# mukteshkrmishra/namazu

Measured on AMD Instinct MI355X. Metric: schedule decisions/sec + trace-pair edit distances/sec at 1/2/4/8 MI355X, higher is better.
Workload: dtype u64; 1 GPU; configs[1] replayable seed sweep; seeds_per_gpu=1048576, events=4096, max_interval_ns=100000000, topk=64, pipeline_streams=3, parallelism=seed-range x1

## Files before the change

### namazu_amd/csrc/replayable.hip

```cpp
#include <algorithm>
#include <cstring>
#include <cstdlib>
#include <numeric>
#include <string>
#include <vector>

#include "nmz_common.h"
#include "nmz_internal.h"
#include "replayable_plan.h"

namespace nmz {

__global__ __launch_bounds__(256) void k_replayable_table(const uint32_t *__restrict__ hoff,
                                                          const uint8_t *__restrict__ hbytes,
                                                          const uint32_t *__restrict__ perm, uint32_t E,
                                                          uint64_t m, int fast, uint4 *__restrict__ table) {
    const uint32_t pos = blockIdx.x;
    const uint32_t L = threadIdx.x;
    const uint32_t e = perm[pos];
    const uint32_t b0 = hoff[e], b1 = hoff[e + 1];
    uint64_t h = L;
    for (uint32_t i = b0; i < b1; ++i) h = fnv_step(h, hbytes[i]);
    const uint64_t C = h - (uint64_t)L * fnv_pow(b1 - b0);
    const uint32_t cm = fast ? (uint32_t)(C % m) : 0u;
// ... 172 lines not shown
    uint64_t h = FNV_OFFSET;
    for (uint32_t i = soff[s], end = soff[s + 1]; i < end; ++i) h = fnv_step(h, sbytes[i]);
    for (uint32_t i = hoff[e], end = hoff[e + 1]; i < end; ++i) h = fnv_step(h, hbytes[i]);
    out[idx] = m ? (int64_t)(h % m) : 0;
}

static bool use_wt(const nmz_replayable_plan *p) {
    return p->wt.on && (replay_oq_enabled() || p->mod.kind != MOD_FAST);
}
static bool use_oq(const nmz_replayable_plan *p) {
    return p->oq.on && (replay_oq_enabled() || p->mod.kind != MOD_FAST);
}

static bool wt_topk_enabled() {
    static const bool on = [] {
        const char *e = ab_env("NMZ_WT_TOPK");
        return !(e && std::string(e) == "0");
    }();
    return on;
}

static int replayable_stats(nmz_replayable_plan *p, hipStream_t st, const uint32_t *d_soff,
                            const uint8_t *d_sbytes, uint64_t S, nmz_sched_stats *d_stats, uint64_t dec_lo = 0,
                            void *wt_topk_scratch = nullptr, uint32_t k = 0,
                            const nmz_replayable_seeds *pre = nullptr) {
    if (S == 0) return NMZ_OK;
    const uint32_t E = p->n_events;
    if (E == 0 || p->mod.kind == MOD_ZERO) {
        hipLaunchKernelGGL(k_stats_constant, dim3(ceil_div(S, 256)), dim3(256), 0, st, S, E, d_stats);
        NMZ_HIP(hipGetLastError());
        return NMZ_OK;
    }
    const bool wt = use_wt(p), stats_kernel = wt || use_oq(p);
    SeedScratch sc;
    if (pre && stats_kernel) {
        sc = pre->sc;
    } else {
        NMZ_CHECK(S <= p->max_seeds, "more seeds than the plan was created for");
        sc = carve_seed_scratch(p->seed_scratch.ptr, p->max_seeds);
        if (pre) {
            NMZ_HIP(hipMemcpyAsync(sc.b.hist, pre->hist, bucket_hist_u32(S) * sizeof(uint32_t),
                                   hipMemcpyDeviceToDevice, st));
            sc.h0 = pre->sc.h0;
        } else {
            NMZ_TRY(seed_prefix_launch(st, d_soff, d_sbytes, dec_lo, S, sc.h0, sc.b.hist));
        }
        if (stats_kernel) NMZ_TRY(bucket_seeds_counted(st, sc.h0, S, OQ_WG, sc.b, sc.counter));
    }
    if (wt) return wt_sweep(p->wt, p->ctx, st, sc.b, p->d_table, E, p->mod, d_stats, S, wt_topk_scratch, k);
    if (stats_kernel) return oq_sweep(p->oq, p->ctx, st, sc.b, p->d_table, E, p->mod, d_stats);
    return pd_sweep(p, st, sc, S, d_stats);
}

static int replayable_run_on(nmz_replayable_plan *p, hipStream_t st, const uint32_t *d_soff, const uint8_t *d_sbytes,
                             uint64_t S, nmz_sched_stats *d_stats, uint64_t seed0, uint32_t k, nmz_topk_entry *d_topk,
                             uint64_t dec_lo, const nmz_replayable_seeds *pre);

static int replayable_run(nmz_replayable_plan *p, hipStream_t st, const uint32_t *d_soff, const uint8_t *d_sbytes,
                          uint64_t S, nmz_sched_stats *d_stats, uint64_t seed0 = 0, uint32_t k = 0,
                          nmz_topk_entry *d_topk = nullptr, uint64_t dec_lo = 0,
                          const nmz_replayable_seeds *pre = nullptr) {
    nmz_replayable_plan::Use *u = nullptr;
    for (auto &x : p->uses)
        if (x.st == st) u = &x;
    if (!u) {
        hipEvent_t ev;
        NMZ_HIP(hipEventCreateWithFlags(&ev, hipEventDisableTiming));
        p->uses.push_back({st, ev});
        u = &p->uses.back();
        if (p->built && st != p->ctx->stream) NMZ_HIP(hipStreamWaitEvent(st, p->built, 0));
    }
    const int rc = replayable_run_on(p, st, d_soff, d_sbytes, S, d_stats, seed0, k, d_topk, dec_lo, pre);
// ... 2 lines not shown
}

static void plan_wait_uses(nmz_replayable_plan *p) {
    for (auto &u : p->uses) {
        (void)hipEventSynchronize(u.ev);
        (void)hipEventDestroy(u.ev);
    }
    p->uses.clear();
    if (p->built) {
        (void)hipEventSynchronize(p->built);
        (void)hipEventDestroy(p->built);
        p->built = nullptr;
    } else {
        (void)hipStreamSynchronize(p->ctx->stream);
    }
}

static int replayable_run_on(nmz_replayable_plan *p, hipStream_t st, const uint32_t *d_soff, const uint8_t *d_sbytes,
                             uint64_t S, nmz_sched_stats *d_stats, uint64_t seed0, uint32_t k, nmz_topk_entry *d_topk,
                             uint64_t dec_lo, const nmz_replayable_seeds *pre) {
    NMZ_CHECK(k <= 256, "top-k supports k <= 256");
    NMZ_CHECK(k == 0 || d_topk, "d_topk is NULL");
    const bool fused = k && k <= 64 && S > 0 && use_wt(p) && wt_topk_enabled();
    if (fused) {
        NMZ_TRY(p->wt_topk.ensure(wt_topk_scratch_bytes(S)));
    }
    NMZ_TRY(replayable_stats(p, st, d_soff, d_sbytes, S, d_stats, dec_lo, fused ? p->wt_topk.ptr : nullptr, k, pre));
    if (fused) {
        const uint32_t *sidx = pre ? pre->sc.b.sorted_idx
                                   : carve_seed_scratch(p->seed_scratch.ptr, p->max_seeds).b.sorted_idx;
        return wt_topk(st, p->wt_topk.ptr, sidx, S, seed0, k, d_topk);
    }
    if (k) {
        NMZ_TRY(p->topk_lists.ensure(topk_scratch_entries(S, k) * sizeof(nmz_topk_entry)));
        NMZ_TRY(topk_select(st, d_stats, S, seed0, k, p->topk_lists.as<nmz_topk_entry>(), d_topk));
    }
    return NMZ_OK;
}

static void plan_destroy_locked(nmz_replayable_plan *plan) {
    plan_wait_uses(plan);
    for (DevBuf *b : plan->buffers()) b->release();
    delete plan;
}

static int plan_create(nmz_ctx *ctx, const uint32_t *hint_off, const uint8_t *hint_bytes, uint32_t E,
                       int64_t max_interval, uint64_t max_seeds, nmz_replayable_plan **out, bool async = false) {
    NMZ_CHECK(ctx && out, "NULL argument");
    NMZ_CHECK(E == 0 || hint_off, "hint_off is NULL");
    *out = nullptr;
    auto *p = new nmz_replayable_plan();
    p->ctx = ctx;
    for (DevBuf *b : p->buffers()) b->pool = &ctx->pool;
    p->n_events = E;
// ... 390 lines not shown
```

### namazu_amd/csrc/replayable_plan.h

```cpp
#pragma once
#include <array>

#include "nmz_common.h"
#include "nmz_internal.h"

namespace nmz {

struct ClassInfo {
    uint64_t pn;
    uint32_t start;
    uint32_t count;
};

constexpr uint32_t REPLAY_SEEDS_PER_UNIT_MIN = 64 * 2;
constexpr uint32_t OQ_WG = 1024;

struct SeedScratch {
    uint64_t *h0;
    Buckets b;
    uint32_t *counter;
};

inline size_t seed_scratch_bytes(uint64_t S) {
    uint64_t max_units = S / REPLAY_SEEDS_PER_UNIT_MIN + 257;
// ... 62 lines not shown
    uint32_t o_mk;
    uint32_t order;
    uint32_t pad;
};
static_assert(sizeof(WtClass) == 64, "WtClass layout");

struct WtPlanHints {
    const uint32_t *hoff;
    const uint8_t *hbytes;
    const uint32_t *perm;
    uint4 *table;
    uint32_t *zero0;
    uint32_t n_zero0;
    uint32_t *zero1;
    uint32_t n_zero1;
};
bool wt_layout(WtState &w, nmz_ctx *ctx, uint32_t E, const ClassInfo *cls, uint32_t n_cls, const ModParams &mod,
               bool fused, std::vector<WtClass> &oc);
int wt_launch(WtState &w, const uint4 *d_table, uint32_t E, const ModParams &mod, hipStream_t st,
              const WtPlanHints *hints, WtClass *d_cls, unsigned long long *d_rowsum, bool sync);
int wt_build(WtState &w, nmz_ctx *ctx, const uint4 *d_table, uint32_t E, const ClassInfo *cls, uint32_t n_cls,
             const ModParams &mod, hipStream_t st);
int wt_sweep(const WtState &w, nmz_ctx *ctx, hipStream_t st, const Buckets &b, const uint4 *d_table, uint32_t E,
             const ModParams &mod, nmz_sched_stats *d_stats, uint64_t S, void *topk_scratch, uint32_t k);
size_t wt_topk_scratch_bytes(uint64_t S);
int wt_topk(hipStream_t st, void *scratch, const uint32_t *sorted_idx, uint64_t S, uint64_t seed0, uint32_t k,
            nmz_topk_entry *d_out);

int pd_sweep(nmz_replayable_plan *p, hipStream_t st, SeedScratch &sc, uint64_t S, nmz_sched_stats *d_stats);

}

struct nmz_replayable_plan {
    nmz_ctx *ctx = nullptr;
    uint32_t n_events = 0;
    int64_t max_interval = 0;
    nmz::ModParams mod{};
    uint32_t n_classes = 0;
    nmz::ClassInfo *d_classes = nullptr;
    uint4 *d_table = nullptr;
    uint32_t *d_hoff = nullptr;
    uint8_t *d_hbytes = nullptr;
    uint64_t max_seeds = 0;
    nmz::DevBuf seed_scratch;
    nmz::DevBuf partial;
    nmz::DevBuf topk_lists;
    nmz::DevBuf plan_mem;
    nmz::OqState oq;
    nmz::WtState wt;
    nmz::DevBuf wt_topk;
// ... 19 lines not shown
```

### namazu_amd/csrc/replayable_wt.hip

```cpp
#include <algorithm>
#include <cstring>
#include <numeric>
#include <cstdlib>
#include <string>
#include <vector>

#include "nmz_common.h"
#include "nmz_internal.h"
#include "replayable_plan.h"

namespace nmz {

#ifndef NMZ_WT_BRUTE
#define NMZ_WT_BRUTE 8
#endif
constexpr uint32_t WT_BRUTE = NMZ_WT_BRUTE;
constexpr uint32_t WT_NMAX = 4096;
constexpr uint32_t WT_LDS_MAX = 160 * 1024 - 256;
constexpr uint32_t WT_NONE = 0xffffffffu;
constexpr uint32_t WT_PAD = 32;
#ifdef WT_BUILD_TRACE
constexpr uint32_t WT_TRACE_PHASES = 10, WT_TRACE_WGS = 8192;
__device__ unsigned long long g_wt_build_trace[WT_TRACE_WGS * WT_TRACE_PHASES];
#define WT_STAMP(k)                                                                                              \
// ... 728 lines not shown
    }
#pragma unroll
    for (int u = 0; u < NS; ++u) {
        const MT vA = MK::load(mk, sA[u] + (sA[u] >> BB) + qA[u]);
        const MT vB = MK::low(MK::inv(MK::load(mk, sB[u] + (sB[u] >> BB) + qB[u])), min(nv - sB[u], BW));
        const uint32_t bA = RA[u] & ~BM, bB = RB[u] & ~BM;
        const uint32_t pA = hitA[u] ? bA + MK::top(belA[u]) : sA[u] + MK::top(vA);
        const uint32_t pB = hitB[u] ? bB + MK::top(belB[u]) : sB[u] + MK::top(vB);
        if (d[u] > 0) {
            const uint32_t t = Hm[u] + cm[pA] - (wrapA[u] ? m : 0u);
            const uint64_t k = ((uint64_t)t << 32) | (0xffffffffu - ev[pA]);
            key[u] = k > key[u] ? k : key[u];
        }
        if (d[u] < n) {
            const uint32_t t = Hm2[u] + cm[pB] - (wrapB[u] ? m : 0u);
            const uint64_t k = ((uint64_t)t << 32) | (0xffffffffu - ev[pB]);
            key[u] = k > key[u] ? k : key[u];
        }
        sum[u] += (uint64_t)d[u] * Hm[u] + (uint64_t)(n - d[u]) * Hm2[u];
    }
}

constexpr uint32_t WT_CAND = 4096;
constexpr uint32_t WT_MAX_GROUPS = 256 * 8;
struct WtTopkState {
    uint32_t n_cand, pad[3];
    unsigned long long gmax[WT_MAX_GROUPS];
    unsigned long long cand_key[WT_CAND];
    unsigned long long cand_idx[WT_CAND];
};

#ifdef WT_TRACE
__device__ unsigned long long g_wt_trace[256][16][10];
#define WT_TSTAMP(slot)                                                                                      \
    do {                                                                                                     \
        if ((threadIdx.x & 63) == 0 && blockIdx.x < 256 && (slot) < 10)                                      \
            g_wt_trace[blockIdx.x][threadIdx.x >> 6][(slot)] = wall_clock64();                               \
    } while (0)
#else
#define WT_TSTAMP(slot) \
    do {                \
    } while (0)
#endif

#ifndef WT_PRIO_TAIL
#define WT_PRIO_TAIL 0
#endif

#ifndef NMZ_WT_WAVES
#define NMZ_WT_WAVES 0
#endif
#if NMZ_WT_WAVES > 0
#define NMZ_WT_ATTR __attribute__((amdgpu_waves_per_eu(NMZ_WT_WAVES, NMZ_WT_WAVES)))
#else
#define NMZ_WT_ATTR
#endif
template <bool BIG, int NS, int BB>
__global__ __launch_bounds__(1024) NMZ_WT_ATTR void k_replayable_sweep_wt(
    const uint32_t *__restrict__ bucket_off, const uint64_t *__restrict__ sorted_h0,
    const uint32_t *__restrict__ sorted_idx, const uint4 *__restrict__ table, uint32_t E,
    const uint4 *__restrict__ blob, uint32_t rb16, const unsigned long long *__restrict__ rowsum,
    const WtClass *__restrict__ classes, uint32_t n_classes, uint32_t m, uint64_t mu, uint32_t m_k64, uint32_t msh,
    uint32_t G, nmz_sched_stats *__restrict__ stats, unsigned long long *__restrict__ span,
    uint64_t *__restrict__ sums, WtTopkState *__restrict__ tk, uint32_t k) {
    constexpr uint32_t CS = 64 * NS;
    extern __shared__ uint4 wt_lds[];
    const uint32_t L = blockIdx.x / G, g = blockIdx.x % G;
    const uint32_t s0 = bucket_off[L], s1 = bucket_off[L + 1];
    const uint32_t nch = (s1 - s0 + CS - 1) / CS;
    const uint32_t c0 = g * nch / G, c1 = (g + 1) * nch / G;
    uint32_t *ctr = reinterpret_cast<uint32_t *>(wt_lds + rb16);
    if (tk && blockIdx.x == 0 && threadIdx.x == 0) tk->n_cand = 0;
    if (c0 == c1) {
        if (tk && threadIdx.x == 0) tk->gmax[blockIdx.x] = 0ull;
        return;
    }
    if (span && threadIdx.x == 0) atomicMax(span, ~(unsigned long long)wall_clock64());
    WT_TSTAMP(9);
    {
        const uint4 *__restrict__ src = blob + (uint64_t)L * rb16;
        constexpr uint32_t B = 8;
        const uint32_t nt = blockDim.x;
        for (uint32_t i0 = 0; i0 < rb16; i0 += B * nt) {
            uint4 v[B];
#pragma unroll
            for (uint32_t k = 0; k < B; ++k) v[k] = src[min(i0 + k * nt + threadIdx.x, rb16 - 1)];
#pragma unroll
            for (uint32_t k = 0; k < B; ++k) wt_lds[min(i0 + k * nt + threadIdx.x, rb16 - 1)] = v[k];
        }
        if (threadIdx.x == 0) {
            *ctr = c0;
            ctr[2] = ctr[3] = 0;
        }
    }
    __syncthreads();
    WT_TSTAMP(0);
#ifdef WT_TRACE
    uint32_t n_done = 0;
#endif
    const char *img = reinterpret_cast<const char *>(wt_lds);
    const uint4 *__restrict__ row = table + (uint64_t)L * E;
    const uint64_t rsum = rowsum[L];
    const uint32_t lane = threadIdx.x & 63;
    WtVConst vc;
#pragma unroll
    for (int r = 0; r < 5; ++r) vc.st4[r] = wt_v(4u << r);
    uint32_t ch = 0;
    if (lane == 0) ch = atomicAdd(ctr, 1u);
    ch = __builtin_amdgcn_readfirstlane(ch);
    uint64_t h0n[NS];
    uint32_t idxn[NS];
#pragma unroll
    for (int u = 0; u < NS; ++u) {
        const uint32_t jn = min(s0 + ch * CS + u * 64 + lane, s1 - 1);
        h0n[u] = sorted_h0[jn];
        idxn[u] = sorted_idx[jn];
    }
    while (ch < c1) {
// ... 11 lines not shown
        uint32_t chn = 0;
        if (lane == 0) chn = atomicAdd(ctr, 1u);
        chn = __builtin_amdgcn_readfirstlane(chn);
#pragma unroll
        for (int u = 0; u < NS; ++u) {
            const uint32_t jn = min(s0 + chn * CS + u * 64 + lane, s1 - 1);
            h0n[u] = sorted_h0[jn];
            idxn[u] = sorted_idx[jn];
        }
        uint64_t sum[NS], key[NS];
        uint32_t W[NS];
#pragma unroll
        for (int u = 0; u < NS; ++u) sum[u] = key[u] = W[u] = 0;
        for (uint32_t c = 0; c < n_classes; ++c)
            wt_seed_class<BIG, NS, BB>(vc, classes[c], img, row, h0, m, mu, m_k64, msh, sum, W, key);
        uint64_t km = 0;
#pragma unroll
        for (int u = 0; u < NS; ++u) {
            const uint32_t j = j0 + u * 64;
            const uint64_t total = sum[u] + rsum - (uint64_t)W[u] * m;
            if (j < s1) {
                const uint64_t kk = total ^ (1ull << 63);
                km = kk > km ? kk : km;
                if (sums) sums[j] = total;
                nmz_sched_stats st;
                st.sum_delay_ns = total;
                st.max_delay_ns = (int64_t)(key[u] >> 32);
                st.argmax_event = ~(uint32_t)key[u];
                st.n_fault = 0;
                st.first_fault = NMZ_NONE;
                st.flags = 0;
                stats[idx[u]] = st;
            }
        }
        if (tk) {
            for (int o = 32; o; o >>= 1) {
                const uint64_t v = __shfl_xor(km, o, 64);
                km = v > km ? v : km;
            }
            if (lane == 0) atomicMax(reinterpret_cast<unsigned long long *>(ctr + 2), (unsigned long long)km);
        }
#ifdef WT_TRACE
        if (++n_done <= 8) WT_TSTAMP(n_done);
#endif
        ch = chn;
    }
    if (span || tk) {
        __syncthreads();
        if (span && threadIdx.x == 0) atomicMax(span + 1, (unsigned long long)wall_clock64());
        if (tk && threadIdx.x == 0) tk->gmax[blockIdx.x] = *reinterpret_cast<const unsigned long long *>(ctr + 2);
    }
}

__device__ __forceinline__ bool wt_better(unsigned long long ka, uint64_t sa, unsigned long long kb, uint64_t sb) {
    return ka > kb || (ka == kb && sa < sb);
}

__global__ __launch_bounds__(256) void k_wt_topk_scan(const uint64_t *__restrict__ sums,
                                                      const uint32_t *__restrict__ sorted_idx, uint64_t S, uint32_t n,
                                                      uint32_t k, WtTopkState *__restrict__ tk) {
    constexpr uint32_t PF = 16;
    constexpr uint32_t NS = 512;
    __shared__ unsigned long long g[NS];
    __shared__ unsigned long long tau_s;
    const uint32_t m = min(n, NS);
    const uint64_t stride = (uint64_t)gridDim.x * 256;
    uint64_t v[PF];
#pragma unroll
    for (uint32_t r = 0; r < PF; ++r) {
        const uint64_t i = (uint64_t)blockIdx.x * 256 + threadIdx.x + r * stride;
        v[r] = i < S ? sums[i] : 0ull;
    }
    for (uint32_t i = threadIdx.x; i < m; i += 256) g[i] = tk->gmax[(uint64_t)i * n / m];
    if (threadIdx.x == 0) tau_s = m >= k ? ~0ull : 0ull;
    __syncthreads();
    if (m >= k) {
        unsigned long long best = ~0ull;
        for (uint32_t i = threadIdx.x; i < m; i += 256) {
            const unsigned long long x = g[i];
            uint32_t gt = 0;
#pragma unroll 8
            for (uint32_t j = 0; j < m; ++j) gt += g[j] > x;
            if (gt < k) best = x < best ? x : best;
        }
        if (best != ~0ull) atomicMin(&tau_s, best);
    }
    __syncthreads();
    const unsigned long long t = tau_s;
    const uint32_t lane = threadIdx.x & 63, w = threadIdx.x >> 6;
    __shared__ uint32_t wsum[4], base_s;
    for (uint64_t i0 = (uint64_t)blockIdx.x * 256; i0 < S; i0 += PF * stride) {
        uint32_t flags = 0;
#pragma unroll
        for (uint32_t r = 0; r < PF; ++r) {
            const uint64_t i = i0 + threadIdx.x + r * stride;
            if (i0 != (uint64_t)blockIdx.x * 256) v[r] = i < S ? sums[i] : 0ull;
            const unsigned long long key = v[r] ^ (1ull << 63);
            flags |= (i < S && key >= t) ? 1u << r : 0u;
        }
        const uint32_t n = __popc(flags);
        uint32_t a = n;
        for (uint32_t d = 1; d < 64; d <<= 1) {
            const uint32_t x = __shfl_up(a, d, 64);
            if (lane >= d) a += x;
        }
        if (lane == 63) wsum[w] = a;
        __syncthreads();
        uint32_t pre = 0, total = 0;
        for (uint32_t x = 0; x < 4; ++x) {
            pre += x < w ? wsum[x] : 0u;
            total += wsum[x];
        }
        if (total) {
            if (threadIdx.x == 0) base_s = atomicAdd(&tk->n_cand, total);
            __syncthreads();
            uint32_t pos = base_s + pre + a - n;
#pragma unroll
            for (uint32_t r = 0; r < PF; ++r) {
                if (flags >> r & 1u) {
                    if (pos < WT_CAND) {
                        const uint64_t i = i0 + threadIdx.x + r * stride;
                        tk->cand_key[pos] = v[r] ^ (1ull << 63);
                        tk->cand_idx[pos] = sorted_idx[i];
                    }
                    ++pos;
                }
            }
        }
        __syncthreads();
    }
}

#ifndef NMZ_WT_SEL_THREADS
#define NMZ_WT_SEL_THREADS 512
#endif
constexpr uint32_t WT_SEL_THREADS = NMZ_WT_SEL_THREADS;
constexpr uint32_t WT_SEL_CHUNK = 2048, WT_SEL_KEEP = (WT_CAND / WT_SEL_CHUNK) * 64;
__global__ __launch_bounds__(WT_SEL_THREADS) void k_wt_topk_select(const uint64_t *__restrict__ sums,
                                                                   const uint32_t *__restrict__ sorted_idx, uint64_t S,
                                                                   uint64_t seed0, uint32_t k,
                                                                   WtTopkState *__restrict__ tk,
                                                                   nmz_topk_entry *__restrict__ out) {
    constexpr uint32_t NT = WT_SEL_THREADS, NW = NT / 64;
    __shared__ unsigned long long ck[WT_SEL_CHUNK];
    __shared__ uint32_t ci[WT_SEL_CHUNK];
    __shared__ unsigned long long sk[WT_SEL_KEEP];
    __shared__ uint32_t si[WT_SEL_KEEP];
    __shared__ unsigned long long bk[NW], bs[NW];
    const uint32_t lane = threadIdx.x & 63;
    const uint32_t c = tk->n_cand;
    auto sentinel = [] {
        nmz_topk_entry e;
        e.seed = UINT64_MAX;
        e.sum_delay_ns = INT64_MIN;
        e.n_fault = 0;
        e.first_fault = NMZ_NONE;
        return e;
    };
    if (c <= WT_CAND) {
        auto sort = [&](uint32_t p2) {
            for (uint32_t kk = 2; kk <= p2; kk <<= 1)
                for (uint32_t j = kk >> 1; j; j >>= 1) {
                    __syncthreads();
                    for (uint32_t i = threadIdx.x; i < p2; i += NT) {
                        const uint32_t l = i ^ j;
                        if (l > i) {
                            const unsigned long long a = ck[i], b = ck[l];
                            const uint32_t ia = ci[i], ib = ci[l];
                            const bool lb = b > a || (b == a && b != 0 && seed0 + ib < seed0 + ia);
                            if (lb == ((i & kk) == 0)) {
                                ck[i] = b;
                                ck[l] = a;
                                ci[i] = ib;
                                ci[l] = ia;
                            }
                        }
                    }
                }
            __syncthreads();
        };
        auto pow2 = [](uint32_t x) {
            uint32_t p = 1;
            while (p < x) p <<= 1;
            return p;
        };
        const uint32_t nch = c > WT_SEL_CHUNK ? (c + WT_SEL_CHUNK - 1) / WT_SEL_CHUNK : 1;
        for (uint32_t q = 0; q < nch; ++q) {
            const uint32_t lo = q * WT_SEL_CHUNK, cc = min(c - lo, WT_SEL_CHUNK), p2 = pow2(cc);
            for (uint32_t i = threadIdx.x; i < p2; i += NT) {
                ck[i] = i < cc ? tk->cand_key[lo + i] : 0ull;
                ci[i] = i < cc ? (uint32_t)tk->cand_idx[lo + i] : ~0u;
            }
            sort(p2);
            if (nch > 1) {
                for (uint32_t i = threadIdx.x; i < k; i += NT) {
                    sk[q * k + i] = ck[i];
                    si[q * k + i] = ci[i];
                }
                __syncthreads();
            }
        }
        if (nch > 1) {
            const uint32_t p2 = pow2(nch * k);
            for (uint32_t i = threadIdx.x; i < p2; i += NT) {
                ck[i] = i < nch * k ? sk[i] : 0ull;
                ci[i] = i < nch * k ? si[i] : ~0u;
            }
            sort(p2);
        }
        for (uint32_t r = threadIdx.x; r < k; r += NT) {
            if (r < c) {
                nmz_topk_entry e;
                e.seed = seed0 + ci[r];
                e.sum_delay_ns = (int64_t)(ck[r] ^ (1ull << 63));
                e.n_fault = 0;
                e.first_fault = NMZ_NONE;
                out[r] = e;
            } else {
                out[r] = sentinel();
            }
        }
    } else {
        unsigned long long pk = ~0ull, ps = 0;
        bool first_rank = true;
        for (uint32_t r = 0; r < k; ++r) {
            unsigned long long mk = 0, ms = ~0ull;
            bool any = false;
            for (uint64_t i = threadIdx.x; i < S; i += NT) {
                const unsigned long long key = sums[i] ^ (1ull << 63), sd = seed0 + sorted_idx[i];
                const bool after = first_rank || wt_better(pk, ps, key, sd);
                if (after && (!any || wt_better(key, sd, mk, ms))) {
                    mk = key;
                    ms = sd;
                    any = true;
                }
            }
            if (!any) mk = 0, ms = ~0ull;
            for (int o = 32; o; o >>= 1) {
                const unsigned long long ok = __shfl_xor(mk, o, 64), os = __shfl_xor(ms, o, 64);
                const bool oany = __shfl_xor((int)any, o, 64);
                if (oany && (!any || wt_better(ok, os, mk, ms))) {
                    mk = ok;
                    ms = os;
                    any = true;
                }
            }
            __syncthreads();
            if (lane == 0) {
                bk[threadIdx.x >> 6] = any ? mk : 0;
                bs[threadIdx.x >> 6] = any ? ms : ~0ull;
                if (!any) bs[threadIdx.x >> 6] = ~0ull, bk[threadIdx.x >> 6] = 0;
            }
            __syncthreads();
            unsigned long long bestk = 0, bests = ~0ull;
            bool found = false;
            for (uint32_t w = 0; w < NW; ++w) {
                const bool real = !(bk[w] == 0 && bs[w] == ~0ull);
                if (real && (!found || wt_better(bk[w], bs[w], bestk, bests))) {
                    bestk = bk[w];
                    bests = bs[w];
                    found = true;
                }
            }
            if (!found) {
                for (uint32_t q = r + threadIdx.x; q < k; q += NT) out[q] = sentinel();
                break;
            }
            if (threadIdx.x == 0) {
                nmz_topk_entry e;
                e.seed = bests;
                e.sum_delay_ns = (int64_t)(bestk ^ (1ull << 63));
                e.n_fault = 0;
                e.first_fault = NMZ_NONE;
                out[r] = e;
            }
            pk = bestk;
            ps = bests;
            first_rank = false;
        }
    }
    __syncthreads();
    if (threadIdx.x == 0) tk->n_cand = 0;
}

static uint32_t bitlen(uint64_t x) {
    uint32_t b = 0;
    while (x) {
        ++b;
        x >>= 1;
    }
    return b;
}

bool wt_enabled() {
    const char *e = ab_env("NMZ_REPLAY_WT");
    return !(e && std::string(e) == "0");
}

static uint32_t wt_groups() {
    static const uint32_t g = [] {
        const char *e = ab_env("NMZ_WT_G");
        const int v = e ? atoi(e) : 1;
        return (uint32_t)((v == 1 || v == 2 || v == 4 || v == 8) ? v : 1);
    }();
    return g;
// ... 45 lines not shown
        o.n = seg[c].count;
        if (o.n <= WT_BRUTE) continue;
        o.K = bitlen(o.n);
        o.nw = o.n / 32 + 1;
        o.o_lv = (uint32_t)off;
        off += r16((uint64_t)wt_levels(o.K, bb) * o.nw * 8);
        o.o_cm = (uint32_t)off;
        off += r16((uint64_t)(o.n + WT_PAD) * 4);
        o.o_chi = (uint32_t)off;
        off += r16((uint64_t)(o.n + WT_PAD) * 4);
        o.o_e = (uint32_t)off;
        off += r16((uint64_t)o.n * 2);
        o.o_im = (uint32_t)off;
        off += r16(257 * 2);
        o.o_ic = (uint32_t)off;
        off += r16(256 * 2);
        o.o_mk = (uint32_t)off;
        off += r16(wt_mask_bytes(o.n, bb));
    }
    return off;
    };
    uint32_t bb = wt_max_bb();
    uint64_t off = layout(bb);
    while (bb > 5 && std::max<uint64_t>(16, r16(off)) + 16 > WT_LDS_MAX) off = layout(--bb);
    {
        std::vector<uint32_t> ord(n_cls);
        std::iota(ord.begin(), ord.end(), 0u);
        std::stable_sort(ord.begin(), ord.end(), [&](uint32_t a, uint32_t b) { return oc[a].n > oc[b].n; });
        for (uint32_t r = 0; r < n_cls; ++r) oc[r].order = ord[r];
    }
    const uint64_t rb = std::max<uint64_t>(16, r16(off));
    if (rb + 16 > WT_LDS_MAX) return false;
    if (!ctx->wt_lds_attr) {
        for (const void *f : {reinterpret_cast<const void *>(k_replayable_sweep_wt<false, 1, 5>),
                              reinterpret_cast<const void *>(k_replayable_sweep_wt<true, 1, 5>),
                              reinterpret_cast<const void *>(k_replayable_sweep_wt<false, 1, 6>),
                              reinterpret_cast<const void *>(k_replayable_sweep_wt<true, 1, 6>),
                              reinterpret_cast<const void *>(k_replayable_sweep_wt<false, 1, 7>),
                              reinterpret_cast<const void *>(k_replayable_sweep_wt<true, 1, 7>),
                              reinterpret_cast<const void *>(k_replayable_wt_build<false, 5>),
                              reinterpret_cast<const void *>(k_replayable_wt_build<true, 5>),
                              reinterpret_cast<const void *>(k_replayable_wt_build<false, 6>),
                              reinterpret_cast<const void *>(k_replayable_wt_build<true, 6>),
                              reinterpret_cast<const void *>(k_replayable_wt_build<false, 7>),
                              reinterpret_cast<const void *>(k_replayable_wt_build<true, 7>)})
            if (hipFuncSetAttribute(f, hipFuncAttributeMaxDynamicSharedMemorySize, (int)WT_LDS_MAX) != hipSuccess) {
                (void)hipGetLastError();
                return false;
            }
        ctx->wt_lds_attr = true;
    }
    w.rb16 = (uint32_t)(rb / 16);
    w.bb = bb;
    w.n_classes = n_cls;
    w.msh = mod.m32 > 255 ? bitlen(mod.m32) - 8 : 0;
// ... 18 lines not shown
                       d_cls, w.msh, bitlen(mod.m32), w.d_blob, w.rb16, d_rowsum, hz);
    NMZ_HIP(hipGetLastError());
    if (sync) NMZ_HIP(hipStreamSynchronize(st));
    w.on = true;
    return NMZ_OK;
}

int wt_build(WtState &w, nmz_ctx *ctx, const uint4 *d_table, uint32_t E, const ClassInfo *cls, uint32_t n_cls,
             const ModParams &mod, hipStream_t st) {
    std::vector<WtClass> oc;
    if (!wt_layout(w, ctx, E, cls, n_cls, mod, false, oc)) return NMZ_OK;
    NMZ_TRY(w.aux.ensure(Carve::bytes_for(256, 8) + Carve::bytes_for(oc.size(), sizeof(WtClass))));
    Carve cv(w.aux.ptr);
    unsigned long long *d_rowsum = cv.take<unsigned long long>(256);
    WtClass *d_cls = cv.take<WtClass>(oc.size());
    NMZ_HIP(hipMemsetAsync(d_rowsum, 0, 256 * 8, st));
    NMZ_TRY(ctx->pin[1].ensure(oc.size() * sizeof(WtClass)));
    std::memcpy(ctx->pin[1].ptr, oc.data(), oc.size() * sizeof(WtClass));
    NMZ_HIP(hipMemcpyAsync(d_cls, ctx->pin[1].ptr, oc.size() * sizeof(WtClass), hipMemcpyHostToDevice, st));
    NMZ_TRY(ctx->pin[1].mark(st));
    return wt_launch(w, d_table, E, mod, st, nullptr, d_cls, d_rowsum, true);
}

size_t wt_topk_scratch_bytes(uint64_t S) {
    return Carve::bytes_for(1, sizeof(WtTopkState)) + Carve::bytes_for(S, 8);
}

int wt_topk(hipStream_t st, void *scratch, const uint32_t *sorted_idx, uint64_t S, uint64_t seed0, uint32_t k,
            nmz_topk_entry *d_out) {
    NMZ_CHECK(k >= 1 && k <= 64, "internal: wt_topk takes 1 <= k <= 64");
    Carve cv(scratch);
    WtTopkState *tk = cv.take<WtTopkState>(1);
    const uint64_t *sums = cv.take<uint64_t>(S);
    const unsigned blocks = (unsigned)std::min<uint64_t>(ceil_div(S, 256), 256);
    hipLaunchKernelGGL(k_wt_topk_scan, dim3(blocks), dim3(256), 0, st, sums, sorted_idx, S, 256 * wt_groups(), k, tk);
    hipLaunchKernelGGL(k_wt_topk_select, dim3(1), dim3(WT_SEL_THREADS), 0, st, sums, sorted_idx, S, seed0, k, tk,
                       d_out);
    NMZ_HIP(hipGetLastError());
    return NMZ_OK;
}

int wt_sweep(const WtState &w, nmz_ctx *ctx, hipStream_t st, const Buckets &b, const uint4 *d_table, uint32_t E,
             const ModParams &mod, nmz_sched_stats *d_stats, uint64_t S, void *topk_scratch, uint32_t k) {
    WtTopkState *tk = nullptr;
    uint64_t *sums = nullptr;
    if (topk_scratch) {
        Carve cv(topk_scratch);
        tk = cv.take<WtTopkState>(1);
        sums = cv.take<uint64_t>(S);
    }
    const uint32_t G = wt_groups(), nt = wt_threads();
    KernelTimer kt(ctx, st, "replayable_sweep");
    unsigned long long *span = kt.span();
    const bool big = mod.m32 >= 0x80000000u;
    auto kern = big ? (w.bb == 7 ? k_replayable_sweep_wt<true, 1, 7>
                       : w.bb == 6 ? k_replayable_sweep_wt<true, 1, 6> : k_replayable_sweep_wt<true, 1, 5>)
                    : (w.bb == 7 ? k_replayable_sweep_wt<false, 1, 7>
                       : w.bb == 6 ? k_replayable_sweep_wt<false, 1, 6> : k_replayable_sweep_wt<false, 1, 5>);
    const size_t lds = w.rb16 * 16u + 16u;
    hipLaunchKernelGGL(kern, dim3(256 * G), dim3(nt), lds, st, b.offset, b.sorted_h0, b.sorted_idx,
                       d_table, E, w.d_blob, w.rb16, w.d_rowsum, static_cast<const WtClass *>(w.d_classes),
                       w.n_classes, mod.m32, mod.mu, mod.m_k64, w.msh, G, d_stats, span, sums, tk, k);
    NMZ_HIP(hipGetLastError());
    return NMZ_OK;
}

}

#ifdef WT_TRACE
extern "C" int nmz_debug_wt_trace(unsigned long long *out) {
    return hipMemcpyFromSymbol(out, HIP_SYMBOL(nmz::g_wt_trace), sizeof(nmz::g_wt_trace)) == hipSuccess ? 0 : -1;
}
#endif

#ifdef WT_BUILD_TRACE
extern "C" int nmz_debug_wt_build_trace(unsigned long long *out, uint32_t n) {
    const uint32_t m = std::min<uint32_t>(n, nmz::WT_TRACE_WGS * nmz::WT_TRACE_PHASES);
    return hipMemcpyFromSymbol(out, HIP_SYMBOL(nmz::g_wt_build_trace), m * 8) == hipSuccess ? 0 : -1;
}
#endif
```

Before: 72250 billion decisions/s.

## Replace per-seed sums scan with per-chunk max records and radix top-k select

The sweep kernel no longer writes a per-seed sums array or keeps per-group maxima. Instead each 64-seed chunk writes one record holding its maximum key, position and count. A single-block selection kernel radix-selects a threshold over the chunk maxima, expands only the qualifying chunks by reading stats, and then sorts the candidates. This removes the separate scan kernel and the S-sized sums write and read, at the cost of a more complex single-block select that could become a serial bottleneck.

```diff
diff --git a/namazu_amd/csrc/replayable.hip b/namazu_amd/csrc/replayable.hip
--- a/namazu_amd/csrc/replayable.hip
+++ b/namazu_amd/csrc/replayable.hip
@@ -218,8 +218,7 @@
 
 static int replayable_stats(nmz_replayable_plan *p, hipStream_t st, const uint32_t *d_soff,
                             const uint8_t *d_sbytes, uint64_t S, nmz_sched_stats *d_stats, uint64_t dec_lo = 0,
-                            void *wt_topk_scratch = nullptr, uint32_t k = 0,
-                            const nmz_replayable_seeds *pre = nullptr) {
+                            void *wt_topk_scratch = nullptr, const nmz_replayable_seeds *pre = nullptr) {
     if (S == 0) return NMZ_OK;
     const uint32_t E = p->n_events;
     if (E == 0 || p->mod.kind == MOD_ZERO) {
@@ -243,7 +242,7 @@
         }
         if (stats_kernel) NMZ_TRY(bucket_seeds_counted(st, sc.h0, S, OQ_WG, sc.b, sc.counter));
     }
-    if (wt) return wt_sweep(p->wt, p->ctx, st, sc.b, p->d_table, E, p->mod, d_stats, S, wt_topk_scratch, k);
+    if (wt) return wt_sweep(p->wt, p->ctx, st, sc.b, p->d_table, E, p->mod, d_stats, S, wt_topk_scratch);
     if (stats_kernel) return oq_sweep(p->oq, p->ctx, st, sc.b, p->d_table, E, p->mod, d_stats);
     return pd_sweep(p, st, sc, S, d_stats);
 }
@@ -292,14 +291,11 @@
     NMZ_CHECK(k <= 256, "top-k supports k <= 256");
     NMZ_CHECK(k == 0 || d_topk, "d_topk is NULL");
     const bool fused = k && k <= 64 && S > 0 && use_wt(p) && wt_topk_enabled();
+    if (fused) NMZ_TRY(p->wt_topk.ensure(wt_topk_scratch_bytes(S)));
+    NMZ_TRY(replayable_stats(p, st, d_soff, d_sbytes, S, d_stats, dec_lo, fused ? p->wt_topk.ptr : nullptr, pre));
     if (fused) {
-        NMZ_TRY(p->wt_topk.ensure(wt_topk_scratch_bytes(S)));
-    }
-    NMZ_TRY(replayable_stats(p, st, d_soff, d_sbytes, S, d_stats, dec_lo, fused ? p->wt_topk.ptr : nullptr, k, pre));
-    if (fused) {
-        const uint32_t *sidx = pre ? pre->sc.b.sorted_idx
-                                   : carve_seed_scratch(p->seed_scratch.ptr, p->max_seeds).b.sorted_idx;
-        return wt_topk(st, p->wt_topk.ptr, sidx, S, seed0, k, d_topk);
+        const Buckets b = pre ? pre->sc.b : carve_seed_scratch(p->seed_scratch.ptr, p->max_seeds).b;
+        return wt_topk(st, p->wt_topk.ptr, b.offset, b.sorted_idx, d_stats, S, seed0, k, d_topk);
     }
     if (k) {
         NMZ_TRY(p->topk_lists.ensure(topk_scratch_entries(S, k) * sizeof(nmz_topk_entry)));
diff --git a/namazu_amd/csrc/replayable_plan.h b/namazu_amd/csrc/replayable_plan.h
--- a/namazu_amd/csrc/replayable_plan.h
+++ b/namazu_amd/csrc/replayable_plan.h
@@ -108,10 +108,10 @@
 int wt_build(WtState &w, nmz_ctx *ctx, const uint4 *d_table, uint32_t E, const ClassInfo *cls, uint32_t n_cls,
              const ModParams &mod, hipStream_t st);
 int wt_sweep(const WtState &w, nmz_ctx *ctx, hipStream_t st, const Buckets &b, const uint4 *d_table, uint32_t E,
-             const ModParams &mod, nmz_sched_stats *d_stats, uint64_t S, void *topk_scratch, uint32_t k);
+             const ModParams &mod, nmz_sched_stats *d_stats, uint64_t S, void *topk_scratch);
 size_t wt_topk_scratch_bytes(uint64_t S);
-int wt_topk(hipStream_t st, void *scratch, const uint32_t *sorted_idx, uint64_t S, uint64_t seed0, uint32_t k,
-            nmz_topk_entry *d_out);
+int wt_topk(hipStream_t st, void *scratch, const uint32_t *bucket_off, const uint32_t *sorted_idx,
+            const nmz_sched_stats *d_stats, uint64_t S, uint64_t seed0, uint32_t k, nmz_topk_entry *d_out);
 
 int pd_sweep(nmz_replayable_plan *p, hipStream_t st, SeedScratch &sc, uint64_t S, nmz_sched_stats *d_stats);
 
diff --git a/namazu_amd/csrc/replayable_wt.hip b/namazu_amd/csrc/replayable_wt.hip
--- a/namazu_amd/csrc/replayable_wt.hip
+++ b/namazu_amd/csrc/replayable_wt.hip
@@ -774,12 +774,15 @@
 }
 
 constexpr uint32_t WT_CAND = 4096;
-constexpr uint32_t WT_MAX_GROUPS = 256 * 8;
+constexpr int WT_NS = 1;
+struct WtChunkRec {
+    unsigned long long key;
+    uint32_t pos, cnt;
+};
+static_assert(sizeof(WtChunkRec) == 16, "WtChunkRec layout");
 struct WtTopkState {
-    uint32_t n_cand, pad[3];
-    unsigned long long gmax[WT_MAX_GROUPS];
     unsigned long long cand_key[WT_CAND];
-    unsigned long long cand_idx[WT_CAND];
+    uint32_t cand_idx[WT_CAND];
 };
 
 #ifdef WT_TRACE
@@ -814,7 +817,7 @@
     const uint4 *__restrict__ blob, uint32_t rb16, const unsigned long long *__restrict__ rowsum,
     const WtClass *__restrict__ classes, uint32_t n_classes, uint32_t m, uint64_t mu, uint32_t m_k64, uint32_t msh,
     uint32_t G, nmz_sched_stats *__restrict__ stats, unsigned long long *__restrict__ span,
-    uint64_t *__restrict__ sums, WtTopkState *__restrict__ tk, uint32_t k) {
+    WtChunkRec *__restrict__ rec) {
     constexpr uint32_t CS = 64 * NS;
     extern __shared__ uint4 wt_lds[];
     const uint32_t L = blockIdx.x / G, g = blockIdx.x % G;
@@ -822,13 +825,12 @@
     const uint32_t nch = (s1 - s0 + CS - 1) / CS;
     const uint32_t c0 = g * nch / G, c1 = (g + 1) * nch / G;
     uint32_t *ctr = reinterpret_cast<uint32_t *>(wt_lds + rb16);
-    if (tk && blockIdx.x == 0 && threadIdx.x == 0) tk->n_cand = 0;
-    if (c0 == c1) {
-        if (tk && threadIdx.x == 0) tk->gmax[blockIdx.x] = 0ull;
-        return;
-    }
+    if (c0 == c1) return;
     if (span && threadIdx.x == 0) atomicMax(span, ~(unsigned long long)wall_clock64());
     WT_TSTAMP(9);
+    uint32_t cb = 0;
+    if (rec)
+        for (uint32_t t = threadIdx.x; t < L; t += blockDim.x) cb += (bucket_off[t + 1] - bucket_off[t] + CS - 1) / CS;
     {
         const uint4 *__restrict__ src = blob + (uint64_t)L * rb16;
         constexpr uint32_t B = 8;
@@ -840,12 +842,15 @@
 #pragma unroll
             for (uint32_t k = 0; k < B; ++k) wt_lds[min(i0 + k * nt + threadIdx.x, rb16 - 1)] = v[k];
         }
-        if (threadIdx.x == 0) {
-            *ctr = c0;
-            ctr[2] = ctr[3] = 0;
+        if (threadIdx.x == 0) *ctr = c0;
+        if (rec && threadIdx.x < 256) {
+            for (int o = 32; o; o >>= 1) cb += __shfl_xor(cb, o, 64);
+            if ((threadIdx.x & 63) == 0) ctr[4 + (threadIdx.x >> 6)] = cb;
+            if (threadIdx.x < 4 && threadIdx.x >= nt / 64) ctr[4 + threadIdx.x] = 0;
         }
     }
     __syncthreads();
+    const uint32_t cbase = rec ? __builtin_amdgcn_readfirstlane(ctr[4] + ctr[5] + ctr[6] + ctr[7]) : 0u;
     WT_TSTAMP(0);
 #ifdef WT_TRACE
     uint32_t n_done = 0;
@@ -903,7 +908,6 @@
             if (j < s1) {
                 const uint64_t kk = total ^ (1ull << 63);
                 km = kk > km ? kk : km;
-                if (sums) sums[j] = total;
                 nmz_sched_stats st;
                 st.sum_delay_ns = total;
                 st.max_delay_ns = (int64_t)(key[u] >> 32);
@@ -914,22 +918,24 @@
                 stats[idx[u]] = st;
             }
         }
-        if (tk) {
+        if (rec) {
             for (int o = 32; o; o >>= 1) {
                 const uint64_t v = __shfl_xor(km, o, 64);
                 km = v > km ? v : km;
             }
-            if (lane == 0) atomicMax(reinterpret_cast<unsigned long long *>(ctr + 2), (unsigned long long)km);
+            const uint32_t p = s0 + ch * CS;
+            if (lane == 0)
+                reinterpret_cast<uint4 *>(rec)[cbase + ch] =
+                    make_uint4((uint32_t)km, (uint32_t)(km >> 32), p, min(CS, s1 - p));
         }
 #ifdef WT_TRACE
         if (++n_done <= 8) WT_TSTAMP(n_done);
 #endif
         ch = chn;
     }
-    if (span || tk) {
+    if (span) {
         __syncthreads();
-        if (span && threadIdx.x == 0) atomicMax(span + 1, (unsigned long long)wall_clock64());
-        if (tk && threadIdx.x == 0) tk->gmax[blockIdx.x] = *reinterpret_cast<const unsigned long long *>(ctr + 2);
+        if (threadIdx.x == 0) atomicMax(span + 1, (unsigned long long)wall_clock64());
     }
 }
 
@@ -937,99 +943,35 @@
     return ka > kb || (ka == kb && sa < sb);
 }
 
-__global__ __launch_bounds__(256) void k_wt_topk_scan(const uint64_t *__restrict__ sums,
-                                                      const uint32_t *__restrict__ sorted_idx, uint64_t S, uint32_t n,
-                                                      uint32_t k, WtTopkState *__restrict__ tk) {
-    constexpr uint32_t PF = 16;
-    constexpr uint32_t NS = 512;
-    __shared__ unsigned long long g[NS];
-    __shared__ unsigned long long tau_s;
-    const uint32_t m = min(n, NS);
-    const uint64_t stride = (uint64_t)gridDim.x * 256;
-    uint64_t v[PF];
-#pragma unroll
-    for (uint32_t r = 0; r < PF; ++r) {
-        const uint64_t i = (uint64_t)blockIdx.x * 256 + threadIdx.x + r * stride;
-        v[r] = i < S ? sums[i] : 0ull;
-    }
-    for (uint32_t i = threadIdx.x; i < m; i += 256) g[i] = tk->gmax[(uint64_t)i * n / m];
-    if (threadIdx.x == 0) tau_s = m >= k ? ~0ull : 0ull;
-    __syncthreads();
-    if (m >= k) {
-        unsigned long long best = ~0ull;
-        for (uint32_t i = threadIdx.x; i < m; i += 256) {
-            const unsigned long long x = g[i];
-            uint32_t gt = 0;
-#pragma unroll 8
-            for (uint32_t j = 0; j < m; ++j) gt += g[j] > x;
-            if (gt < k) best = x < best ? x : best;
-        }
-        if (best != ~0ull) atomicMin(&tau_s, best);
-    }
-    __syncthreads();
-    const unsigned long long t = tau_s;
-    const uint32_t lane = threadIdx.x & 63, w = threadIdx.x >> 6;
-    __shared__ uint32_t wsum[4], base_s;
-    for (uint64_t i0 = (uint64_t)blockIdx.x * 256; i0 < S; i0 += PF * stride) {
-        uint32_t flags = 0;
-#pragma unroll
-        for (uint32_t r = 0; r < PF; ++r) {
-            const uint64_t i = i0 + threadIdx.x + r * stride;
-            if (i0 != (uint64_t)blockIdx.x * 256) v[r] = i < S ? sums[i] : 0ull;
-            const unsigned long long key = v[r] ^ (1ull << 63);
-            flags |= (i < S && key >= t) ? 1u << r : 0u;
-        }
-        const uint32_t n = __popc(flags);
-        uint32_t a = n;
-        for (uint32_t d = 1; d < 64; d <<= 1) {
-            const uint32_t x = __shfl_up(a, d, 64);
-            if (lane >= d) a += x;
-        }
-        if (lane == 63) wsum[w] = a;
-        __syncthreads();
-        uint32_t pre = 0, total = 0;
-        for (uint32_t x = 0; x < 4; ++x) {
-            pre += x < w ? wsum[x] : 0u;
-            total += wsum[x];
-        }
-        if (total) {
-            if (threadIdx.x == 0) base_s = atomicAdd(&tk->n_cand, total);
-            __syncthreads();
-            uint32_t pos = base_s + pre + a - n;
-#pragma unroll
-            for (uint32_t r = 0; r < PF; ++r) {
-                if (flags >> r & 1u) {
-                    if (pos < WT_CAND) {
-                        const uint64_t i = i0 + threadIdx.x + r * stride;
-                        tk->cand_key[pos] = v[r] ^ (1ull << 63);
-                        tk->cand_idx[pos] = sorted_idx[i];
-                    }
-                    ++pos;
-                }
-            }
-        }
-        __syncthreads();
-    }
-}
-
 #ifndef NMZ_WT_SEL_THREADS
 #define NMZ_WT_SEL_THREADS 512
 #endif
-constexpr uint32_t WT_SEL_THREADS = NMZ_WT_SEL_THREADS;
+#ifndef NMZ_WT_SEL_KPT
+#define NMZ_WT_SEL_KPT 33
+#endif
+constexpr uint32_t WT_SEL_THREADS = NMZ_WT_SEL_THREADS, WT_SEL_KPT = NMZ_WT_SEL_KPT;
 constexpr uint32_t WT_SEL_CHUNK = 2048, WT_SEL_KEEP = (WT_CAND / WT_SEL_CHUNK) * 64;
-__global__ __launch_bounds__(WT_SEL_THREADS) void k_wt_topk_select(const uint64_t *__restrict__ sums,
-                                                                   const uint32_t *__restrict__ sorted_idx, uint64_t S,
-                                                                   uint64_t seed0, uint32_t k,
-                                                                   WtTopkState *__restrict__ tk,
+template <uint32_t CS>
+__global__ __launch_bounds__(WT_SEL_THREADS) __attribute__((amdgpu_waves_per_eu(4))) void k_wt_topk_chunks(const uint32_t *__restrict__ bucket_off,
+                                                                   const WtChunkRec *__restrict__ rec,
+                                                                   const uint32_t *__restrict__ sorted_idx,
+                                                                   const nmz_sched_stats *__restrict__ stats,
+                                                                   uint64_t S, uint64_t seed0, uint32_t k,
+                                                                   uint32_t nmax, WtTopkState *__restrict__ tk,
                                                                    nmz_topk_entry *__restrict__ out) {
-    constexpr uint32_t NT = WT_SEL_THREADS, NW = NT / 64;
+    constexpr uint32_t NT = WT_SEL_THREADS, NW = NT / 64, KPT = WT_SEL_KPT;
+    static_assert(NT >= 256 && NT % 64 == 0 && CS <= 65535 && 2 * WT_SEL_CHUNK == WT_CAND, "selection layout");
     __shared__ unsigned long long ck[WT_SEL_CHUNK];
     __shared__ uint32_t ci[WT_SEL_CHUNK];
     __shared__ unsigned long long sk[WT_SEL_KEEP];
     __shared__ uint32_t si[WT_SEL_KEEP];
     __shared__ unsigned long long bk[NW], bs[NW];
-    const uint32_t lane = threadIdx.x & 63;
-    const uint32_t c = tk->n_cand;
+    __shared__ uint32_t hist[256];
+    __shared__ uint32_t wtot[NW], sel[2], cnt_s[2];
+    uint32_t *fpos = reinterpret_cast<uint32_t *>(ck);
+    uint16_t *fcnt = reinterpret_cast<uint16_t *>(ci);
+    const uint32_t tid = threadIdx.x, lane = tid & 63, wave = tid >> 6;
+    const unsigned long long below = (1ull << lane) - 1ull;
     auto sentinel = [] {
         nmz_topk_entry e;
         e.seed = UINT64_MAX;
@@ -1038,6 +980,162 @@
         e.first_fault = NMZ_NONE;
         return e;
     };
+    __builtin_amdgcn_s_setprio(3);
+    unsigned long long kreg[KPT];
+#pragma unroll
+    for (uint32_t r = 0; r < KPT; ++r) {
+        const uint32_t i = tid + r * NT;
+        kreg[r] = i < nmax ? rec[i].key : 0ull;
+    }
+    const unsigned long long k0 = rec[0].key;
+    {
+        uint32_t v = tid < 256 ? (bucket_off[tid + 1] - bucket_off[tid] + CS - 1) / CS : 0u;
+        for (int o = 32; o; o >>= 1) v += __shfl_xor(v, o, 64);
+        if (lane == 0) wtot[wave] = v;
+        if (tid < 2) cnt_s[tid] = 0;
+    }
+    __syncthreads();
+    const uint32_t n = wtot[0] + wtot[1] + wtot[2] + wtot[3];
+    const bool all = n < k;
+    unsigned long long tau = 0;
+    uint32_t hb = 0;
+    if (!all) {
+        unsigned long long diff = 0;
+#pragma unroll
+        for (uint32_t r = 0; r < KPT; ++r) diff |= tid + r * NT < n ? kreg[r] ^ k0 : 0ull;
+        for (uint32_t i = tid + KPT * NT; i < n; i += NT) diff |= rec[i].key ^ k0;
+        for (int o = 32; o; o >>= 1) diff |= __shfl_xor(diff, o, 64);
+        if (lane == 0) bk[wave] = diff;
+        __syncthreads();
+        diff = 0;
+        for (uint32_t w = 0; w < NW; ++w) diff |= bk[w];
+        hb = diff ? 64u - (uint32_t)__clzll(diff) : 0u;
+    }
+    const uint32_t sh0 = hb > 32 ? hb - 32 : 0;
+    uint32_t w32[KPT], t32 = 0;
+#pragma unroll
+    for (uint32_t r = 0; r < KPT; ++r) w32[r] = (uint32_t)(kreg[r] >> sh0);
+    if (!all) {
+        uint32_t sh = min(hb, 32u), kk = k;
+        uint32_t pref = sh >= 32 ? 0u : ((uint32_t)(k0 >> sh0) >> sh) << sh;
+        while (sh) {
+            const uint32_t hi = sh, w = min(8u, sh);
+            sh -= w;
+            const uint32_t dm = (1u << w) - 1u;
+            if (tid < 256) hist[tid] = 0;
+            __syncthreads();
+            uint32_t cur = 0, cnt = 0;
+            auto add = [&](uint32_t key) {
+                if (hi >= 32 || (key >> hi) == (pref >> hi)) {
+                    const uint32_t d = (key >> sh) & dm;
+                    if (d != cur && cnt) {
+                        atomicAdd(&hist[cur], cnt);
+                        cnt = 0;
+                    }
+                    cur = d;
+                    ++cnt;
+                }
+            };
+#pragma unroll
+            for (uint32_t r = 0; r < KPT; ++r)
+                if (tid + r * NT < n) add(w32[r]);
+            for (uint32_t i = tid + KPT * NT; i < n; i += NT) add((uint32_t)(rec[i].key >> sh0));
+            if (cnt) atomicAdd(&hist[cur], cnt);
+            __syncthreads();
+            uint32_t c = 0, inc = 0;
+            if (tid < 256) {
+                c = inc = hist[255 - tid];
+                for (int o = 1; o < 64; o <<= 1) {
+                    const uint32_t v = __shfl_up(inc, o, 64);
+                    if (lane >= (uint32_t)o) inc += v;
+                }
+                if (lane == 63) wtot[wave] = inc;
+            }
+            __syncthreads();
+            if (tid < 256) {
+                for (uint32_t x = 0; x < wave; ++x) inc += wtot[x];
+                if (inc - c < kk && kk <= inc) {
+                    sel[0] = 255 - tid;
+                    sel[1] = kk - (inc - c);
+                }
+            }
+            __syncthreads();
+            pref |= sel[0] << sh;
+            kk = sel[1];
+        }
+        t32 = pref;
+        tau = (sh0 + 32 >= 64 ? 0ull : (k0 >> (sh0 + 32)) << (sh0 + 32)) | ((unsigned long long)pref << sh0);
+    }
+    {
+        static_assert(KPT <= 64, "one mark bit per register key");
+        auto list = [&](uint32_t i) {
+            const uint32_t slot = atomicAdd(&cnt_s[0], 1u);
+            if (slot < WT_CAND) {
+                fpos[slot] = rec[i].pos;
+                fcnt[slot] = (uint16_t)rec[i].cnt;
+            }
+        };
+        unsigned long long fm = 0;
+#pragma unroll
+        for (uint32_t r = 0; r < KPT; ++r) fm |= (tid + r * NT < n && (all || w32[r] >= t32)) ? 1ull << r : 0ull;
+        while (fm) {
+            const uint32_t r = (uint32_t)__ffsll((long long)fm) - 1u;
+            fm &= fm - 1ull;
+            list(tid + r * NT);
+        }
+        for (uint32_t i = tid + KPT * NT; i < n; i += NT)
+            if (all || (uint32_t)(rec[i].key >> sh0) >= t32) list(i);
+    }
+    __syncthreads();
+    const uint32_t nf = cnt_s[0];
+    constexpr uint32_t U = 16;
+    const uint32_t items = nf * CS;
+    const bool one = nf <= WT_CAND && items <= U * NT;
+    uint32_t idx[U], slot[U], fl = 0;
+    unsigned long long key[U];
+    if (nf <= WT_CAND) {
+        for (uint32_t i0 = 0; i0 < items; i0 += U * NT) {
+            bool ok[U];
+            fl = 0;
+#pragma unroll
+            for (uint32_t u = 0; u < U; ++u) {
+                const uint32_t it = i0 + u * NT + tid, fi = min(it / CS, nf - 1), o = it % CS;
+                ok[u] = it < items && o < fcnt[fi];
+                idx[u] = ok[u] ? sorted_idx[fpos[fi] + o] : 0u;
+            }
+#pragma unroll
+            for (uint32_t u = 0; u < U; ++u) key[u] = ok[u] ? stats[idx[u]].sum_delay_ns ^ (1ull << 63) : 0ull;
+#pragma unroll
+            for (uint32_t u = 0; u < U; ++u) {
+                const bool f = ok[u] && key[u] >= tau;
+                const unsigned long long mask = __ballot(f);
+                slot[u] = 0;
+                if (mask) {
+                    uint32_t base = 0;
+                    if (lane == 0) base = atomicAdd(&cnt_s[1], (uint32_t)__popcll(mask));
+                    base = __builtin_amdgcn_readfirstlane(base);
+                    slot[u] = base + (uint32_t)__popcll(mask & below);
+                    fl |= f ? 1u << u : 0u;
+                    if (!one && f && slot[u] < WT_CAND) {
+                        tk->cand_key[slot[u]] = key[u];
+                        tk->cand_idx[slot[u]] = idx[u];
+                    }
+                }
+            }
+        }
+        __syncthreads();
+    }
+    const uint32_t c = nf <= WT_CAND ? cnt_s[1] : WT_CAND + 1;
+    const bool direct = one && c <= WT_SEL_CHUNK;
+    if (one && !direct && c <= WT_CAND) {
+#pragma unroll
+        for (uint32_t u = 0; u < U; ++u)
+            if (fl >> u & 1u) {
+                tk->cand_key[slot[u]] = key[u];
+                tk->cand_idx[slot[u]] = idx[u];
+            }
+        __syncthreads();
+    }
     if (c <= WT_CAND) {
         auto sort = [&](uint32_t p2) {
             for (uint32_t kk = 2; kk <= p2; kk <<= 1)
@@ -1068,9 +1166,22 @@
         const uint32_t nch = c > WT_SEL_CHUNK ? (c + WT_SEL_CHUNK - 1) / WT_SEL_CHUNK : 1;
         for (uint32_t q = 0; q < nch; ++q) {
             const uint32_t lo = q * WT_SEL_CHUNK, cc = min(c - lo, WT_SEL_CHUNK), p2 = pow2(cc);
-            for (uint32_t i = threadIdx.x; i < p2; i += NT) {
-                ck[i] = i < cc ? tk->cand_key[lo + i] : 0ull;
-                ci[i] = i < cc ? (uint32_t)tk->cand_idx[lo + i] : ~0u;
+            if (direct) {
+                for (uint32_t i = cc + threadIdx.x; i < p2; i += NT) {
+                    ck[i] = 0ull;
+                    ci[i] = ~0u;
+                }
+#pragma unroll
+                for (uint32_t u = 0; u < U; ++u)
+                    if (fl >> u & 1u) {
+                        ck[slot[u]] = key[u];
+                        ci[slot[u]] = idx[u];
+                    }
+            } else {
+                for (uint32_t i = threadIdx.x; i < p2; i += NT) {
+                    ck[i] = i < cc ? tk->cand_key[lo + i] : 0ull;
+                    ci[i] = i < cc ? tk->cand_idx[lo + i] : ~0u;
+                }
             }
             sort(p2);
             if (nch > 1) {
@@ -1108,7 +1219,7 @@
             unsigned long long mk = 0, ms = ~0ull;
             bool any = false;
             for (uint64_t i = threadIdx.x; i < S; i += NT) {
-                const unsigned long long key = sums[i] ^ (1ull << 63), sd = seed0 + sorted_idx[i];
+                const unsigned long long key = stats[i].sum_delay_ns ^ (1ull << 63), sd = seed0 + i;
                 const bool after = first_rank || wt_better(pk, ps, key, sd);
                 if (after && (!any || wt_better(key, sd, mk, ms))) {
                     mk = key;
@@ -1130,7 +1241,6 @@
             if (lane == 0) {
                 bk[threadIdx.x >> 6] = any ? mk : 0;
                 bs[threadIdx.x >> 6] = any ? ms : ~0ull;
-                if (!any) bs[threadIdx.x >> 6] = ~0ull, bk[threadIdx.x >> 6] = 0;
             }
             __syncthreads();
             unsigned long long bestk = 0, bests = ~0ull;
@@ -1160,8 +1270,6 @@
             first_rank = false;
         }
     }
-    __syncthreads();
-    if (threadIdx.x == 0) tk->n_cand = 0;
 }
 
 static uint32_t bitlen(uint64_t x) {
@@ -1253,7 +1361,7 @@
     };
     uint32_t bb = wt_max_bb();
     uint64_t off = layout(bb);
-    while (bb > 5 && std::max<uint64_t>(16, r16(off)) + 16 > WT_LDS_MAX) off = layout(--bb);
+    while (bb > 5 && std::max<uint64_t>(16, r16(off)) + 32 > WT_LDS_MAX) off = layout(--bb);
     {
         std::vector<uint32_t> ord(n_cls);
         std::iota(ord.begin(), ord.end(), 0u);
@@ -1261,7 +1369,7 @@
         for (uint32_t r = 0; r < n_cls; ++r) oc[r].order = ord[r];
     }
     const uint64_t rb = std::max<uint64_t>(16, r16(off));
-    if (rb + 16 > WT_LDS_MAX) return false;
+    if (rb + 32 > WT_LDS_MAX) return false;
     if (!ctx->wt_lds_attr) {
         for (const void *f : {reinterpret_cast<const void *>(k_replayable_sweep_wt<false, 1, 5>),
                               reinterpret_cast<const void *>(k_replayable_sweep_wt<true, 1, 5>),
@@ -1326,45 +1434,43 @@
     return wt_launch(w, d_table, E, mod, st, nullptr, d_cls, d_rowsum, true);
 }
 
+static uint64_t wt_max_chunks(uint64_t S) { return S / (64 * WT_NS) + 256; }
 size_t wt_topk_scratch_bytes(uint64_t S) {
-    return Carve::bytes_for(1, sizeof(WtTopkState)) + Carve::bytes_for(S, 8);
-}
-
-int wt_topk(hipStream_t st, void *scratch, const uint32_t *sorted_idx, uint64_t S, uint64_t seed0, uint32_t k,
-            nmz_topk_entry *d_out) {
+    return Carve::bytes_for(1, sizeof(WtTopkState)) + Carve::bytes_for(wt_max_chunks(S), sizeof(WtChunkRec));
+}
+
+int wt_topk(hipStream_t st, void *scratch, const uint32_t *bucket_off, const uint32_t *sorted_idx,
+            const nmz_sched_stats *d_stats, uint64_t S, uint64_t seed0, uint32_t k, nmz_topk_entry *d_out) {
     NMZ_CHECK(k >= 1 && k <= 64, "internal: wt_topk takes 1 <= k <= 64");
     Carve cv(scratch);
     WtTopkState *tk = cv.take<WtTopkState>(1);
-    const uint64_t *sums = cv.take<uint64_t>(S);
-    const unsigned blocks = (unsigned)std::min<uint64_t>(ceil_div(S, 256), 256);
-    hipLaunchKernelGGL(k_wt_topk_scan, dim3(blocks), dim3(256), 0, st, sums, sorted_idx, S, 256 * wt_groups(), k, tk);
-    hipLaunchKernelGGL(k_wt_topk_select, dim3(1), dim3(WT_SEL_THREADS), 0, st, sums, sorted_idx, S, seed0, k, tk,
-                       d_out);
+    const WtChunkRec *rec = cv.take<WtChunkRec>(wt_max_chunks(S));
+    hipLaunchKernelGGL(k_wt_topk_chunks<64 * WT_NS>, dim3(1), dim3(WT_SEL_THREADS), 0, st, bucket_off, rec, sorted_idx,
+                       d_stats, S, seed0, k, (uint32_t)wt_max_chunks(S), tk, d_out);
     NMZ_HIP(hipGetLastError());
     return NMZ_OK;
 }
 
 int wt_sweep(const WtState &w, nmz_ctx *ctx, hipStream_t st, const Buckets &b, const uint4 *d_table, uint32_t E,
-             const ModParams &mod, nmz_sched_stats *d_stats, uint64_t S, void *topk_scratch, uint32_t k) {
-    WtTopkState *tk = nullptr;
-    uint64_t *sums = nullptr;
+             const ModParams &mod, nmz_sched_stats *d_stats, uint64_t S, void *topk_scratch) {
+    WtChunkRec *rec = nullptr;
     if (topk_scratch) {
         Carve cv(topk_scratch);
-        tk = cv.take<WtTopkState>(1);
-        sums = cv.take<uint64_t>(S);
+        cv.take<WtTopkState>(1);
+        rec = cv.take<WtChunkRec>(wt_max_chunks(S));
     }
     const uint32_t G = wt_groups(), nt = wt_threads();
     KernelTimer kt(ctx, st, "replayable_sweep");
     unsigned long long *span = kt.span();
     const bool big = mod.m32 >= 0x80000000u;
-    auto kern = big ? (w.bb == 7 ? k_replayable_sweep_wt<true, 1, 7>
-                       : w.bb == 6 ? k_replayable_sweep_wt<true, 1, 6> : k_replayable_sweep_wt<true, 1, 5>)
-                    : (w.bb == 7 ? k_replayable_sweep_wt<false, 1, 7>
-                       : w.bb == 6 ? k_replayable_sweep_wt<false, 1, 6> : k_replayable_sweep_wt<false, 1, 5>);
-    const size_t lds = w.rb16 * 16u + 16u;
+    auto kern = big ? (w.bb == 7 ? k_replayable_sweep_wt<true, WT_NS, 7>
+                       : w.bb == 6 ? k_replayable_sweep_wt<true, WT_NS, 6> : k_replayable_sweep_wt<true, WT_NS, 5>)
+                    : (w.bb == 7 ? k_replayable_sweep_wt<false, WT_NS, 7>
+                       : w.bb == 6 ? k_replayable_sweep_wt<false, WT_NS, 6> : k_replayable_sweep_wt<false, WT_NS, 5>);
+    const size_t lds = w.rb16 * 16u + 32u;
     hipLaunchKernelGGL(kern, dim3(256 * G), dim3(nt), lds, st, b.offset, b.sorted_h0, b.sorted_idx,
                        d_table, E, w.d_blob, w.rb16, w.d_rowsum, static_cast<const WtClass *>(w.d_classes),
-                       w.n_classes, mod.m32, mod.mu, mod.m_k64, w.msh, G, d_stats, span, sums, tk, k);
+                       w.n_classes, mod.m32, mod.mu, mod.m_k64, w.msh, G, d_stats, span, rec);
     NMZ_HIP(hipGetLastError());
     return NMZ_OK;
 }
```

Measured after the change: 78470 billion decisions/s (median of 6 runs). 1.09x the previous value.
